# locuslab/qpth

Hardware: NVIDIA H100
Metric: QPs/sec (fwd+bwd) batch=128 nz=100 nineq=100 (higher is better)
Workload: dtype f64

## Files before the change

qpth_b200/csrc/qp_alt.cu:

```cuda
#include <cuda_runtime.h>
#include <math.h>
#include <stdint.h>
#include <string.h>

#include <mutex>

#include "../../include/qpth_b200.h"
#ifndef QPB_NT
#error "compile with -DQPB_NT=192|512 -DQPB_ALT_CTAS=3|1"
#endif
#define QPB_NS_CAT2(a, b) a##b
#define QPB_NS_CAT(a, b) QPB_NS_CAT2(a, b)
#define qpb QPB_NS_CAT(qpb_nt, QPB_NT)
#include "qp_solve.cuh"
#include "qp_setup_pf.cuh"

extern "C" void qpb200_internal_cuda_error(int err, const char* what);

namespace {

constexpr int kAltCtas = QPB_ALT_CTAS;
constexpr int kMin = (kAltCtas > 1) ? kAltCtas : 0;

KDims alt_dims(const qpb200_plan* p) {
    KDims D;
    D.n = p->nz; D.m = p->nineq; D.e = p->neq; D.ep = p->neq_pad; D.ms = p->ms; D.msp = p->ms_pad;
    D.ldw = p->ldw; D.lds = p->lds; D.rows_s = p->rows_s; D.vl = p->vl;
    D.lp = (int)p->L_elems;
    D.reg = 0.0;
    return D;
}

std::mutex g_mu;
template <typename K>
int alt_set_smem(K kernel, size_t bytes, size_t* cur) {
    int dev = 0;
    cudaError_t e = cudaGetDevice(&dev);
    if (e != cudaSuccess) { qpb200_internal_cuda_error((int)e, "cudaGetDevice"); return QPB200_ERR_CUDA; }
    std::lock_guard<std::mutex> lock(g_mu);
    if (dev < 16 && cur[dev] >= bytes) return QPB200_OK;
    e = cudaFuncSetAttribute(kernel, cudaFuncAttributeMaxDynamicSharedMemorySize, (int)bytes);
    if (e != cudaSuccess) { qpb200_internal_cuda_error((int)e, "cudaFuncSetAttribute"); return QPB200_ERR_CUDA; }
    if (dev < 16) cur[dev] = bytes;
    return QPB200_OK;
}
int alt_check_launch() {
    cudaError_t e = cudaGetLastError();
    if (e != cudaSuccess) { qpb200_internal_cuda_error((int)e, "kernel launch (qp_alt.cu)"); return QPB200_ERR_CUDA; }
    return QPB200_OK;
}
size_t g_fwd[16], g_kkt[16], g_bwd[16];

}

#define QPB_CAT2(a, b, c) a##b##c
#define QPB_CAT(a, b, c) QPB_CAT2(a, b, c)
#define QPB_ALT_NAME(fn) QPB_CAT(qpb200_alt, QPB_NT, fn)

extern "C" {

int QPB_ALT_NAME(_forward)(const qpb200_plan* plan, size_t smem, int nbatch, const double* p, int64_t sp, const double* h,
                           int64_t sh, const double* b, int64_t sb, const double* Lfac, const double* Wfac,
                           const double* Kfac, int sF, double eps, double stall_tol, double best_tie, int notImprovedLim,
                           int maxIter, double* zhat, double* lam, double* slacks, double* nus, int* iters,
                           double* best_resid, double* trace, void* stream) {
    cudaStream_t st = (cudaStream_t)stream;
    const KDims D = alt_dims(plan);
    int rc = alt_set_smem(k_forward_fast<true, true, kMin>, smem, g_fwd);
    if (rc) return rc;
    k_forward_fast<true, true, kMin><<<nbatch, qpb::fast::kNT, smem, st>>>(
        D, p, sp, h, sh, b, sb, Lfac, Wfac, Kfac, sF, eps, stall_tol, best_tie, notImprovedLim, maxIter, zhat, lam,
        slacks, nus, iters, best_resid, trace);
    return alt_check_launch();
}

int QPB_ALT_NAME(_forward_res)(const qpb200_plan* plan, size_t smem, int nbatch, const double* p, int64_t sp, const double* h,
                               int64_t sh, const double* b, int64_t sb, const double* Lfac, const double* Wfac,
                               const double* Kfac, int sF, double eps, double stall_tol, double best_tie, int notImprovedLim,
                               int maxIter, double* zhat, double* lam, double* slacks, double* nus, int* iters,
                               double* best_resid, double* trace, void* stream) {
#if QPB_NT == 512
    cudaStream_t st = (cudaStream_t)stream;
    const KDims D = alt_dims(plan);
    static size_t cur[16];
    int rc = alt_set_smem(k_forward_fast<false, true, 0>, smem, cur);
    if (rc) return rc;
    k_forward_fast<false, true, 0><<<nbatch, qpb::fast::kNT, smem, st>>>(
        D, p, sp, h, sh, b, sb, Lfac, Wfac, Kfac, sF, eps, stall_tol, best_tie, notImprovedLim, maxIter, zhat, lam,
        slacks, nus, iters, best_resid, trace);
    return alt_check_launch();
#else
    (void)plan; (void)smem; (void)nbatch; (void)p; (void)sp; (void)h; (void)sh; (void)b; (void)sb; (void)Lfac; (void)Wfac;
    (void)Kfac; (void)sF; (void)eps; (void)stall_tol; (void)best_tie; (void)notImprovedLim; (void)maxIter; (void)zhat;
    (void)lam; (void)slacks; (void)nus; (void)iters; (void)best_resid; (void)trace; (void)stream;
    return QPB200_ERR_BAD_ARG;
#endif
}

int QPB_ALT_NAME(_solve_kkt)(const qpb200_plan* plan, size_t smem, int nbatch, const double* d, const double* rx,
                             const double* rs, const double* rz, const double* ry, const double* Lfac, const double* Wfac,
                             const double* Kfac, int sF, double* dx, double* ds, double* dz, double* dy, void* stream) {
    cudaStream_t st = (cudaStream_t)stream;
    const KDims D = alt_dims(plan);
    BwdOut O;
    memset(&O, 0, sizeof(O));
    int rc = alt_set_smem(k_kkt_fast<false, true, true, kMin>, smem, g_kkt);
    if (rc) return rc;
    k_kkt_fast<false, true, true, kMin><<<nbatch, qpb::fast::kNT, smem, st>>>(
        D, d, rx, rs, rz, ry, nullptr, nullptr, nullptr, nullptr, Lfac, Wfac, Kfac, sF, dx, ds, dz, dy, O);
    return alt_check_launch();
}

#if QPB_NT == 192
int QPB_ALT_NAME(_setup)(const qpb200_plan* plan, size_t smem, int nsys, const double* Q, int64_t sQ, const double* G,
                         int64_t sG, const double* A, int64_t sA, double reg, double* Lfac, double* Wfac, double* Kfac,
                         int* spd_flag, void* stream) {
    static size_t g_setup[16];
    cudaStream_t st = (cudaStream_t)stream;
    KDims D = alt_dims(plan);
    D.reg = reg;
    int rc = alt_set_smem(k_setup_pf<kMin>, smem, g_setup);
    if (rc) return rc;
    k_setup_pf<kMin><<<nsys, qpb::fast::kNT, smem, st>>>(D, Q, sQ, G, sG, A, sA, Lfac, Wfac, Kfac, spd_flag);
    return alt_check_launch();
}
#endif

int QPB_ALT_NAME(_backward)(const qpb200_plan* plan, size_t smem, int nbatch, const double* dl_dzhat,
                            const double* dl_dlam, const double* dl_dnu, const double* zhat,
                            const double* lam, const double* slacks, const double* nus, const double* Lfac,
                            const double* Wfac, const double* Kfac, int sF, double* dQ, int mean_Q, double* dp, int mean_p,
                            double* dG, int mean_G, double* dh, int mean_h, double* dA, int mean_A, double* db, int mean_b,
                            double* dxv, double* dlamv, double* dnuv, void* stream) {
    cudaStream_t st = (cudaStream_t)stream;
    const KDims D = alt_dims(plan);
    BwdOut O;
    O.dQ = dQ; O.dp = dp; O.dG = dG; O.dh = dh; O.dA = dA; O.db = db;
    O.mQ = mean_Q; O.mp = mean_p; O.mG = mean_G; O.mh = mean_h; O.mA = mean_A; O.mb = mean_b;
    int rc = alt_set_smem(k_kkt_fast<true, true, true, kMin>, smem, g_bwd);
    if (rc) return rc;
    k_kkt_fast<true, true, true, kMin><<<nbatch, qpb::fast::kNT, smem, st>>>(
        D, nullptr, dl_dzhat, nullptr, dl_dlam, dl_dnu, zhat, lam, slacks, nus, Lfac, Wfac, Kfac, sF, dxv, nullptr,
        dlamv, dnuv, O);
    return alt_check_launch();
}

}
```

qpth_b200/csrc/qp_fast.cuh:

```cuda
#pragma once
#include "qp_device.cuh"

namespace qpb {
namespace fast {

#define QPB_SMEM extern __shared__ __align__(16) double qsm[]

#ifdef QPB_TIMING
__device__ long long g_cta[4 * 8192];
__device__ int g_tim_target = 0;
__device__ __forceinline__ long long gtimer() { long long t; asm volatile("mov.u64 %0, %globaltimer;" : "=l"(t)); return t; }
__device__ __forceinline__ int smid() { int r; asm volatile("mov.u32 %0, %smid;" : "=r"(r)); return r; }
__device__ long long g_tim[128];
__shared__ long long s_tim[129];
#define QPB_TICK(i)                                                         \
    do {                                                                    \
        if (threadIdx.x == 0) {                                             \
            const long long _t = clock64();                                 \
            s_tim[i] += _t - s_tim[128];                                    \
            s_tim[128] = _t;                                                \
        }                                                                   \
    } while (0)
__shared__ long long s_tim2;
#define QPB_TICK1(i)                                                        \
    do {                                                                    \
        if (threadIdx.x == 32) {                                            \
            const long long _t = clock64();                                 \
            s_tim[i] += _t - s_tim2;                                        \
            s_tim2 = _t;                                                    \
        }                                                                   \
    } while (0)
#else
#define QPB_TICK(i) do {} while (0)
#define QPB_TICK1(i) do {} while (0)
#endif

#ifndef QPB_NT
#define QPB_NT 256
#endif
constexpr int kNT = QPB_NT;


__device__ __forceinline__ void f_load_lower8(const double* Mb, int ld, double (&Lk)[36]) {
#pragma unroll
    for (int r = 0; r < 8; ++r)
#pragma unroll
        for (int c = 0; c <= r; c += 2) {
            const double2 v = *reinterpret_cast<const double2*>(Mb + r * ld + c);
            Lk[QPB_LIDX(r, c)] = v.x;
            if (c + 1 <= r) Lk[QPB_LIDX(r, c + 1)] = v.y;
        }
}

__device__ __forceinline__ double f_rsqrt(double x) {
    double y;
    asm("rsqrt.approx.ftz.f64 %0, %1;" : "=d"(y) : "d"(x));
    const double t = x * y;
    const double e = fma(-t, y, 1.0);
    const double p = fma(0.375, e, 0.5);
    const double ye = y * e;
    return fma(ye, p, y);
}

__device__ __forceinline__ void f_factor8_regs(double (&Lk)[36]) {
#pragma unroll
    for (int c = 0; c < 8; ++c) {
        const double ri = f_rsqrt(Lk[QPB_LIDX(c, c)]);
        Lk[QPB_LIDX(c, c)] = ri;
#pragma unroll
        for (int r = c + 1; r < 8; ++r) Lk[QPB_LIDX(r, c)] *= ri;
#pragma unroll
        for (int r = c + 1; r < 8; ++r)
#pragma unroll
            for (int cc = c + 1; cc <= r; ++cc)
                Lk[QPB_LIDX(r, cc)] = fma(-Lk[QPB_LIDX(r, c)], Lk[QPB_LIDX(cc, c)], Lk[QPB_LIDX(r, cc)]);
    }
}
__device__ __forceinline__ void f_store_lower8(double* Mb, int ld, const double (&Lk)[36]) {
#pragma unroll
    for (int r = 0; r < 8; ++r)
#pragma unroll
        for (int c = 0; c <= r; c += 2)
            *reinterpret_cast<double2*>(Mb + r * ld + c) =
                make_double2(Lk[QPB_LIDX(r, c)], (c + 1 <= r) ? Lk[QPB_LIDX(r, c + 1)] : 0.0);
}

__device__ __forceinline__ void f_row_solve8(double (&a)[8], const double (&Lk)[36]) {
#pragma unroll
    for (int c = 0; c < 8; ++c) {
        a[c] *= Lk[QPB_LIDX(c, c)];
#pragma unroll
        for (int c2 = c + 1; c2 < 8; ++c2) a[c2] = fma(-a[c], Lk[QPB_LIDX(c2, c)], a[c2]);
    }
}

__device__ __forceinline__ void f_ld8(const double* p, double (&a)[8]) {
    const double2 v0 = *reinterpret_cast<const double2*>(p), v1 = *reinterpret_cast<const double2*>(p + 2),
                  v2 = *reinterpret_cast<const double2*>(p + 4), v3 = *reinterpret_cast<const double2*>(p + 6);
    a[0] = v0.x; a[1] = v0.y; a[2] = v1.x; a[3] = v1.y; a[4] = v2.x; a[5] = v2.y; a[6] = v3.x; a[7] = v3.y;
}
__device__ __forceinline__ void f_st8(double* p, const double (&a)[8]) {
    *reinterpret_cast<double2*>(p) = make_double2(a[0], a[1]);
    *reinterpret_cast<double2*>(p + 2) = make_double2(a[2], a[3]);
    *reinterpret_cast<double2*>(p + 4) = make_double2(a[4], a[5]);
    *reinterpret_cast<double2*>(p + 6) = make_double2(a[6], a[7]);
}

__device__ __forceinline__ void named_bar_sync(int id, int count) {
    asm volatile("bar.sync %0, %1;" ::"r"(id), "r"(count) : "memory");
}
__device__ __forceinline__ void named_bar_arrive(int id, int count) {
    asm volatile("bar.arrive %0, %1;" ::"r"(id), "r"(count) : "memory");
}

__device__ __noinline__ void f_chol_chain(int A, int ld, int n, int c0) {
    QPB_SMEM;
    const int lane = threadIdx.x & 31;
    const int g = lane >> 2, q = lane & 3;
    const int nts = (n - c0) >> 3;
    double* M = qsm + A;
    double Lk[36];
    for (int k = -1; k < nts; ++k) {
        const int k0 = c0 + 8 * k;
        if (k >= 0 && k + 1 < nts) {
            if (lane < 8) {
                double a[8];
                double* rowp = M + (k0 + 8 + lane) * ld + k0;
                f_ld8(rowp, a);
                f_row_solve8(a, Lk);
                f_st8(rowp, a);
            }
            __syncwarp();
            named_bar_arrive(1, kNT);
            QPB_TICK(96 + k);
            double* pd = M + (k0 + 8 + g) * ld + k0 + 8 + 2 * q;
            const double* pr = M + (k0 + 8 + g) * ld + k0 + q;
            double2 cv = *reinterpret_cast<const double2*>(pd);
            const double a0 = pr[0], a1 = pr[4];
            dmma884(cv.x, cv.y, -a0, a0);
            dmma884(cv.x, cv.y, -a1, a1);
            *reinterpret_cast<double2*>(pd) = cv;
            __syncwarp();
            QPB_TICK(24);
        }
        if (k + 1 < nts) {
            f_load_lower8(M + (k0 + 8) * ld + k0 + 8, ld, Lk);
            __syncwarp();
            f_factor8_regs(Lk);
            if (lane == 0) f_store_lower8(M + (k0 + 8) * ld + k0 + 8, ld, Lk);
            if (k >= 0) QPB_TICK(80 + k);
        }
        QPB_TICK(26);
        __syncthreads();
        if (k >= 0) QPB_TICK(112 + k);
    }
}

__device__ __noinline__ void f_chol_update(int A, int ld, int n, int c0, int aug, int tabo) {
    QPB_SMEM;
    const int tid = threadIdx.x, lane = tid & 31, warp = tid >> 5;
    const int g = lane >> 2, q = lane & 3;
    const int nts = (n - c0) >> 3;
    const int noff = (nts * (nts - 1)) / 2;
    const uint16_t* tab = reinterpret_cast<const uint16_t*>(qsm + tabo);
    double* M = qsm + A;
    const int uw = (warp == 4) ? -1 : (warp < 4 ? warp - 1 : warp - 2);
    double C[kCholMaxOff][2];
    int tt_of[kCholMaxOff];
    const int gq = (c0 + g) * ld + q;
    if (uw >= 0) {
#pragma unroll
        for (int s = 0; s < kCholMaxOff; ++s) {
            const int idx = s * 6 + uw;
            const bool ok = idx < noff;
            const int tt = ok ? tab[idx] : 0;
            tt_of[s] = ok ? tt : -1;
            const double2 v = ok ? *reinterpret_cast<const double2*>(M + gq + q + 8 * (tt >> 8) * ld + c0 + 8 * (tt & 255))
                                 : make_double2(0.0, 0.0);
            C[s][0] = v.x; C[s][1] = v.y;
        }
    }
    __syncthreads();
    for (int k = 0; k < nts; ++k) {
        const int k0 = c0 + 8 * k;
        const bool last = (k + 1 >= nts);
        QPB_TICK1(40);
        {
            const int t = tid - 32;
            const int nrows = n - k0 - 16;
            const int naug = nrows > 0 ? nrows : 0;
            if (t <= naug) {
                double Ls[36], a[8];
                double* rowp = (t < naug) ? (M + (k0 + 16 + t) * ld + k0) : (qsm + aug + k0);
                f_ld8(rowp, a);
                f_load_lower8(M + k0 * ld + k0, ld, Ls);
                f_row_solve8(a, Ls);
                f_st8(rowp, a);
            }
        }
        QPB_TICK1(64 + k);
        if (!last) {
            named_bar_sync(1, kNT);
            QPB_TICK1(42);
            if (uw >= 0) {
#pragma unroll
                for (int s = kCholMaxOff - 1; s >= 0; s -= 2) {
                    const int s1 = s, s2 = (s - 1 >= 0) ? s - 1 : 0;
                    const int t1 = tt_of[s1], t2 = tt_of[s2];
                    const bool act1 = (t1 & 255) > k && t1 >= 0;
                    const bool act2 = (s - 1 >= 0) && (t2 & 255) > k && t2 >= 0;
                    if (!act1 && !act2) continue;
                    const double* pa1 = M + gq + 8 * (t1 >> 8) * ld + k0;
                    const double* pb1 = M + gq + 8 * (t1 & 255) * ld + k0;
                    const double* pa2 = M + gq + 8 * (t2 >> 8) * ld + k0;
                    const double* pb2 = M + gq + 8 * (t2 & 255) * ld + k0;
                    double a10 = 0, a11 = 0, b10 = 0, b11 = 0, a20 = 0, a21 = 0, b20 = 0, b21 = 0;
                    if (act1) { a10 = pa1[0]; a11 = pa1[4]; b10 = pb1[0]; b11 = pb1[4]; }
                    if (act2) { a20 = pa2[0]; a21 = pa2[4]; b20 = pb2[0]; b21 = pb2[4]; }
                    if (act1) dmma884(C[s1][0], C[s1][1], -a10, b10);
                    if (act2) dmma884(C[s2][0], C[s2][1], -a20, b20);
                    if (act1) dmma884(C[s1][0], C[s1][1], -a11, b11);
                    if (act2) dmma884(C[s2][0], C[s2][1], -a21, b21);
                    if (act1 && (t1 & 255) == k + 1)
                        *reinterpret_cast<double2*>(M + gq + q + 8 * (t1 >> 8) * ld + c0 + 8 * (k + 1)) = make_double2(C[s1][0], C[s1][1]);
                    if (act2 && (t2 & 255) == k + 1)
                        *reinterpret_cast<double2*>(M + gq + q + 8 * (t2 >> 8) * ld + c0 + 8 * (k + 1)) = make_double2(C[s2][0], C[s2][1]);
                }
                for (int s = k + 2 + uw; s < nts; s += 6) {
                    double* pd = M + (c0 + 8 * s + g) * ld + c0 + 8 * s + 2 * q;
                    const double* pr = M + (c0 + 8 * s + g) * ld + k0 + q;
                    double2 cv = *reinterpret_cast<const double2*>(pd);
                    const double a0 = pr[0], a1 = pr[4];
                    dmma884(cv.x, cv.y, -a0, a0);
                    dmma884(cv.x, cv.y, -a1, a1);
                    *reinterpret_cast<double2*>(pd) = cv;
                }
            } else {
                double y[8];
                f_ld8(qsm + aug + k0, y);
                for (int j = k0 + 8 + lane; j < n; j += 32) {
                    double pr[8];
                    f_ld8(M + j * ld + k0, pr);
                    double acc0 = qsm[aug + j], acc1 = 0.0;
#pragma unroll
                    for (int c = 0; c < 8; c += 2) { acc0 = fma(-pr[c], y[c], acc0); acc1 = fma(-pr[c + 1], y[c + 1], acc1); }
                    qsm[aug + j] = acc0 + acc1;
                }
            }
        }
        QPB_TICK1(48 + k);
        __syncthreads();
        QPB_TICK1(44);
    }
}

__device__ __forceinline__ void f_chol(int A, int ld, int n, int c0, int aug, int tabo) {
    if (threadIdx.x < 32) f_chol_chain(A, ld, n, c0);
    else f_chol_update(A, ld, n, c0, aug, tabo);
}

__device__ __noinline__ void f_trsv_fwd(int A, int ld, int n, int kbeg, int kend, int b, int u) {
    QPB_SMEM;
    const int tid = threadIdx.x;
    const double* M = qsm + A;
    for (int k0 = kbeg; k0 < kend; k0 += 8) {
        const int nbelow = n - k0 - 8;
        if (tid < nbelow || tid == 0) {
            double Lk[36], y[8], row[8];
            const bool has = tid < nbelow;
            f_ld8(qsm + b + k0, y);
            if (has) f_ld8(M + (k0 + 8 + tid) * ld + k0, row);
            f_load_lower8(M + k0 * ld + k0, ld, Lk);
            double acc0 = has ? qsm[b + k0 + 8 + tid] : 0.0, acc1 = 0.0;
#pragma unroll
            for (int c = 0; c < 8; ++c) {
                y[c] *= Lk[QPB_LIDX(c, c)];
#pragma unroll
                for (int c2 = c + 1; c2 < 8; ++c2) y[c2] = fma(-y[c], Lk[QPB_LIDX(c2, c)], y[c2]);
                if (has) { if (c & 1) acc1 = fma(-row[c], y[c], acc1); else acc0 = fma(-row[c], y[c], acc0); }
            }
            if (tid == 0) f_st8(qsm + u + k0, y);
            if (has) qsm[b + k0 + 8 + tid] = acc0 + acc1;
        }
        __syncthreads();
    }
}

__device__ __noinline__ void f_trsv_bwd(int A, int ld, int n, int u, int w) {
    QPB_SMEM;
    const int tid = threadIdx.x;
    const double* M = qsm + A;
    for (int k0 = n - 8; k0 >= 0; k0 -= 8) {
        if (tid < k0 || tid == 0) {
            double Lk[36], y[8];
            const bool has = tid < k0;
            f_ld8(qsm + u + k0, y);
            double col[8];
            if (has) {
#pragma unroll
                for (int c = 0; c < 8; ++c) col[c] = M[(k0 + c) * ld + tid];
            }
            f_load_lower8(M + k0 * ld + k0, ld, Lk);
            double acc0 = has ? qsm[u + tid] : 0.0, acc1 = 0.0;
#pragma unroll
            for (int c = 7; c >= 0; --c) {
                y[c] *= Lk[QPB_LIDX(c, c)];
#pragma unroll
                for (int c2 = 0; c2 < c; ++c2) y[c2] = fma(-y[c], Lk[QPB_LIDX(c, c2)], y[c2]);
                if (has) { if (c & 1) acc1 = fma(-col[c], y[c], acc1); else acc0 = fma(-col[c], y[c], acc0); }
            }
            if (tid == 0) f_st8(qsm + w + k0, y);
            if (has) qsm[u + tid] = acc0 + acc1;
        }
        __syncthreads();
    }
}

__device__ __noinline__ void f_invert8(int Mb_off, int ld) {
    QPB_SMEM;
    double* Mb = qsm + Mb_off;
    if ((threadIdx.x & 31) == 0) {
        double Lk[36], T[36];
        f_load_lower8(Mb, ld, Lk);
#pragma unroll
        for (int c = 0; c < 8; ++c) {
            T[QPB_LIDX(c, c)] = Lk[QPB_LIDX(c, c)];
#pragma unroll
            for (int r = c + 1; r < 8; ++r) {
                double sacc = 0.0;
#pragma unroll
                for (int j = c; j < r; ++j) sacc = fma(Lk[QPB_LIDX(r, j)], T[QPB_LIDX(j, c)], sacc);
                T[QPB_LIDX(r, c)] = -Lk[QPB_LIDX(r, r)] * sacc;
            }
        }
#pragma unroll
        for (int r = 1; r < 8; ++r)
#pragma unroll
            for (int c = 0; c < r; ++c) Mb[c * ld + r] = T[QPB_LIDX(r, c)];
    }
    __syncwarp();
}

__device__ __noinline__ void f_rows_times_LinvT(int A, int ld, int n, int Wm, int ldw, int rt) {
    QPB_SMEM;
    const int lane = threadIdx.x & 31, g = lane >> 2, q = lane & 3;
    const double* M = qsm + A;
    double* Wp = qsm + Wm + (8 * rt + g) * ldw;
    const int nct = n >> 3;
    for (int j = 0; j < nct; ++j) {
        double2 cv = *reinterpret_cast<const double2*>(Wp + 8 * j + 2 * q);
        const double* pb = M + (8 * j + g) * ld + q;
        for (int i = 0; i < j; ++i) {
            const double a0 = Wp[8 * i + q], a1 = Wp[8 * i + 4 + q];
            const double b0 = pb[8 * i], b1 = pb[8 * i + 4];
            dmma884(cv.x, cv.y, -a0, b0);
            dmma884(cv.x, cv.y, -a1, b1);
        }
        *reinterpret_cast<double2*>(Wp + 8 * j + 2 * q) = cv;
        __syncwarp();
        const double a0 = Wp[8 * j + q], a1 = Wp[8 * j + 4 + q];
        const double* Tb = M + (8 * j) * ld + 8 * j;
        const int c0 = q, c1 = 4 + q;
        const double b0 = (c0 < g) ? Tb[c0 * ld + g] : (c0 == g ? Tb[g * ld + g] : 0.0);
        const double b1 = (c1 < g) ? Tb[c1 * ld + g] : (c1 == g ? Tb[g * ld + g] : 0.0);
        double d0 = 0.0, d1 = 0.0;
        dmma884(d0, d1, a0, b0);
        dmma884(d0, d1, a1, b1);
        __syncwarp();
        *reinterpret_cast<double2*>(Wp + 8 * j + 2 * q) = make_double2(d0, d1);
        __syncwarp();
    }
}

__device__ __noinline__ void f_whiten(int Lp, int n, int dinvL, int b, int u) {
    QPB_SMEM;
    trsv_fwd(qsm + Lp, PackedIdx{}, n, 0, n, qsm + dinvL, qsm + b, qsm + u, (int)threadIdx.x, kNT);
}
__device__ __noinline__ void f_unwhiten(int Lp, int n, int dinvL, int u, int w) {
    QPB_SMEM;
    trsv_bwd(qsm + Lp, PackedIdx{}, n, qsm + dinvL, qsm + u, qsm + w, (int)threadIdx.x, kNT);
}

template <bool kTwo>
__device__ __forceinline__ void f_matvec_rows_impl(int W, int ld, int rows, int cols, int x1, int x2, int y1, int y2) {
    QPB_SMEM;
    const int tid = threadIdx.x, h = tid & 1;
    for (int rb = 0; rb < rows; rb += kNT / 2) {
        const int r = rb + (tid >> 1);
        const bool ok = r < rows;
        const double* a = qsm + W + (ok ? r : 0) * ld + 2 * h;
        double s1a = 0.0, s1b = 0.0, s2a = 0.0, s2b = 0.0;
#pragma unroll 2
        for (int c = 2 * h; c < cols; c += 4, a += 4) {
            const double2 w = *reinterpret_cast<const double2*>(a);
            const double2 u = *reinterpret_cast<const double2*>(qsm + x1 + c);
            const bool hi = c + 1 < cols;
            const double wy = hi ? w.y : 0.0;
            s1a = fma(w.x, u.x, s1a); s1b = fma(wy, hi ? u.y : 0.0, s1b);
            if (kTwo) {
                const double2 v = *reinterpret_cast<const double2*>(qsm + x2 + c);
                s2a = fma(w.x, v.x, s2a); s2b = fma(wy, hi ? v.y : 0.0, s2b);
            }
        }
        double s1 = s1a + s1b, s2 = s2a + s2b;
        __syncwarp();
        s1 += __shfl_xor_sync(0xffffffffu, s1, 1);
        if (kTwo) s2 += __shfl_xor_sync(0xffffffffu, s2, 1);
        if (ok && h == 0) {
            qsm[y1 + r] = s1;
            if (kTwo) qsm[y2 + r] = s2;
        }
    }
}
__device__ __noinline__ void f_matvec_rows2(int W, int ld, int rows, int cols, int x1, int x2, int y1, int y2) {
    f_matvec_rows_impl<true>(W, ld, rows, cols, x1, x2, y1, y2);
}
__device__ __noinline__ void f_matvec_rows1(int W, int ld, int rows, int cols, int x1, int y1) {
    f_matvec_rows_impl<false>(W, ld, rows, cols, x1, 0, y1, 0);
}
__device__ __noinline__ void f_matvec_cols(int W, int ld, int rows, int cols, int v, int p0, int p1, int out,
                                           int a, double sa, int b, double sgn) {
    QPB_SMEM;
    const int tid = threadIdx.x;
    const int half = kNT / 2;
    const int gidx = tid / half, c = tid - gidx * half;
    const int chunk = (rows + 1) >> 1;
    for (int c0 = 0; c0 < cols; c0 += half) {
        const int cc = c0 + c;
        if (cc < cols) {
            const int r0 = gidx * chunk, r1 = min(rows, r0 + chunk);
            const double* Wp = qsm + W + cc;
            double s0 = 0.0, s1 = 0.0, s2 = 0.0, s3 = 0.0;
            int r = r0;
#pragma unroll 1
            for (; r + 3 < r1; r += 4) {
                s0 = fma(Wp[(r + 0) * ld], qsm[v + r + 0], s0);
                s1 = fma(Wp[(r + 1) * ld], qsm[v + r + 1], s1);
                s2 = fma(Wp[(r + 2) * ld], qsm[v + r + 2], s2);
                s3 = fma(Wp[(r + 3) * ld], qsm[v + r + 3], s3);
            }
#pragma unroll 1
            for (; r < r1; ++r) s0 = fma(Wp[r * ld], qsm[v + r], s0);
            qsm[(gidx ? p1 : p0) + cc] = (s0 + s1) + (s2 + s3);
        }
    }
    __syncthreads();
    for (int cc = tid; cc < cols; cc += kNT) {
        double r = sa * qsm[a + cc] + sgn * (qsm[p0 + cc] + qsm[p1 + cc]);
        if (b >= 0) r += qsm[b + cc];
        qsm[out + cc] = r;
    }
    __syncthreads();
}

__device__ __forceinline__ void f_cols2_out(int c, double wdv, double wv, int xt, int rxt, int pt, double alpha) {
    QPB_SMEM;
    const double dx = -qsm[rxt + c] - wdv;
    const double x = fma(alpha, dx, qsm[xt + c]);
    qsm[xt + c] = x;
    qsm[rxt + c] = (x + wv) + qsm[pt + c];
}
__device__ __noinline__ void f_matvec_cols2(int W, int ld, int rows, int cols, int dv, int v, int p0, int p1, int p2,
                                            int p3, int xt, int rxt, int pt, double alpha) {
    QPB_SMEM;
    const int tid = threadIdx.x;
    const int half = kNT / 2;
    const int gidx = tid / half, c = tid - gidx * half;
    const int chunk = (rows + 1) >> 1;
    for (int c0 = 0; c0 < cols; c0 += half) {
        const int cc = c0 + c;
        if (cc < cols) {
            const int r0 = gidx * chunk, r1 = min(rows, r0 + chunk);
            const double* Wp = qsm + W + cc;
            double s0 = 0.0, s1 = 0.0, s2 = 0.0, s3 = 0.0, u0 = 0.0, u1 = 0.0, u2 = 0.0, u3 = 0.0;
            int r = r0;
#pragma unroll 1
            for (; r + 3 < r1; r += 4) {
                const double w0 = Wp[(r + 0) * ld], w1 = Wp[(r + 1) * ld], w2 = Wp[(r + 2) * ld], w3 = Wp[(r + 3) * ld];
                s0 = fma(w0, qsm[dv + r + 0], s0); u0 = fma(w0, qsm[v + r + 0], u0);
                s1 = fma(w1, qsm[dv + r + 1], s1); u1 = fma(w1, qsm[v + r + 1], u1);
                s2 = fma(w2, qsm[dv + r + 2], s2); u2 = fma(w2, qsm[v + r + 2], u2);
                s3 = fma(w3, qsm[dv + r + 3], s3); u3 = fma(w3, qsm[v + r + 3], u3);
            }
#pragma unroll 1
            for (; r < r1; ++r) {
                const double w0 = Wp[r * ld];
                s0 = fma(w0, qsm[dv + r], s0); u0 = fma(w0, qsm[v + r], u0);
            }
            qsm[(gidx ? p1 : p0) + cc] = (s0 + s1) + (s2 + s3);
            qsm[(gidx ? p3 : p2) + cc] = (u0 + u1) + (u2 + u3);
        }
    }
    __syncthreads();
    for (int cc = tid; cc < cols; cc += kNT)
        f_cols2_out(cc, qsm[p0 + cc] + qsm[p1 + cc], qsm[p2 + cc] + qsm[p3 + cc], xt, rxt, pt, alpha);
    __syncthreads();
}

__device__ __noinline__ double f_tri_norm2(int Lp, int n, int x) {
    QPB_SMEM;
    const int tid = threadIdx.x, q4 = tid >> 2, l = tid & 3;
    double acc = 0.0;
    const int npairs = (n + 1) >> 1;
    for (int pb = 0; pb < npairs; pb += kNT / 4) {
        const int pi = pb + q4;
        const bool act = pi < npairs;
        const int ra = act ? pi : 0, rb = n - 1 - ra;
        const double* La = qsm + Lp + (ra * (ra + 1)) / 2;
        const double* Lb = qsm + Lp + (rb * (rb + 1)) / 2;
        double sa = 0.0, sb = 0.0;
        if (act) {
#pragma unroll 2
            for (int c = l; c <= ra; c += 4) sa = fma(La[c], qsm[x + c], sa);
            if (rb != ra) {
#pragma unroll 2
                for (int c = l; c <= rb; c += 4) sb = fma(Lb[c], qsm[x + c], sb);
            }
        }
        __syncwarp();
        sa += __shfl_xor_sync(0xffffffffu, sa, 1); sb += __shfl_xor_sync(0xffffffffu, sb, 1);
        sa += __shfl_xor_sync(0xffffffffu, sa, 2); sb += __shfl_xor_sync(0xffffffffu, sb, 2);
        if (l == 0) acc = fma(sa, sa, fma(sb, sb, acc));
    }
    return acc;
}

__device__ __forceinline__ double2 ldg2(const double* p) { return __ldg(reinterpret_cast<const double2*>(p)); }

template <bool kTwo>
__device__ __forceinline__ void g_matvec_rows_impl(const double* __restrict__ Wg, int ld, int rows, int cols, int x1,
                                                   int x2, int y1, int y2) {
    QPB_SMEM;
    constexpr int kRG = kNT / 8;
    const int tid = threadIdx.x, j = tid & 7, rg = kRG - 1 - (tid >> 3);
#pragma unroll 1
    for (int rb = 0; rb < rows; rb += 2 * kRG) {
        const int r0 = rb + rg, r1 = r0 + kRG;
        const bool ok0 = r0 < rows, ok1 = r1 < rows;
        const double* p0 = Wg + (size_t)(ok0 ? r0 : 0) * ld;
        const double* p1 = Wg + (size_t)(ok1 ? r1 : 0) * ld;
        double a0 = 0.0, a1 = 0.0, b0 = 0.0, b1 = 0.0;
#pragma unroll 1
        for (int cb = 2 * j; cb < cols; cb += 112) {
            double2 w0[7], w1[7];
#pragma unroll
            for (int k = 0; k < 7; ++k) {
                const int c = cb + 16 * k;
                const bool in = c < cols;
                w0[k] = in ? ldg2(p0 + c) : make_double2(0.0, 0.0);
                w1[k] = in ? ldg2(p1 + c) : make_double2(0.0, 0.0);
            }
#pragma unroll
            for (int k = 0; k < 7; ++k) {
                const int c = cb + 16 * k;
                if (c < cols) {
                    const bool hi = c + 1 < cols;
                    double2 u = *reinterpret_cast<const double2*>(qsm + x1 + c);
                    if (!hi) u.y = 0.0;
                    const double wy0 = hi ? w0[k].y : 0.0, wy1 = hi ? w1[k].y : 0.0;
                    a0 = fma(w0[k].x, u.x, a0); a0 = fma(wy0, u.y, a0);
                    b0 = fma(w1[k].x, u.x, b0); b0 = fma(wy1, u.y, b0);
                    if (kTwo) {
                        double2 v = *reinterpret_cast<const double2*>(qsm + x2 + c);
                        if (!hi) v.y = 0.0;
                        a1 = fma(w0[k].x, v.x, a1); a1 = fma(wy0, v.y, a1);
                        b1 = fma(w1[k].x, v.x, b1); b1 = fma(wy1, v.y, b1);
                    }
                }
            }
        }
        __syncwarp();
#pragma unroll
        for (int o = 1; o < 8; o <<= 1) {
            a0 += __shfl_xor_sync(0xffffffffu, a0, o);
            b0 += __shfl_xor_sync(0xffffffffu, b0, o);
            if (kTwo) {
                a1 += __shfl_xor_sync(0xffffffffu, a1, o);
                b1 += __shfl_xor_sync(0xffffffffu, b1, o);
            }
        }
        if (j == 0) {
            if (ok0) { qsm[y1 + r0] = a0; if (kTwo) qsm[y2 + r0] = a1; }
            if (ok1) { qsm[y1 + r1] = b0; if (kTwo) qsm[y2 + r1] = b1; }
        }
    }
}
__device__ __noinline__ void g_matvec_rows2(const double* __restrict__ Wg, int ld, int rows, int cols, int x1, int x2,
                                            int y1, int y2) {
    g_matvec_rows_impl<true>(Wg, ld, rows, cols, x1, x2, y1, y2);
}
__device__ __noinline__ void g_matvec_rows1(const double* __restrict__ Wg, int ld, int rows, int cols, int x1, int y1) {
    g_matvec_rows_impl<false>(Wg, ld, rows, cols, x1, 0, y1, 0);
}

__device__ __noinline__ void g_matvec_cols(const double* __restrict__ Wg, int ld, int rows, int cols, int v, int out,
                                           int a, double sa, int b, double sgn) {
    QPB_SMEM;
    const int tid = threadIdx.x, lane = tid & 31, warp = tid >> 5, g = lane >> 3, cq = lane & 7;
#pragma unroll 1
    for (int c0 = 0; c0 < cols; c0 += 16 * (kNT / 32)) {
        const int c = c0 + 16 * warp + 2 * cq;
        const bool okc = c < cols;
        const double* pc = Wg + (okc ? c : 0);
        double s0 = 0.0, s1 = 0.0;
#pragma unroll 1
        for (int rb = g; rb < rows; rb += 4 * 13) {
            double2 w[13];
#pragma unroll
            for (int k = 0; k < 13; ++k) {
                const int r = rb + 4 * k;
                w[k] = (r < rows) ? ldg2(pc + (size_t)r * ld) : make_double2(0.0, 0.0);
            }
#pragma unroll
            for (int k = 0; k < 13; ++k) {
                const int r = rb + 4 * k;
                if (r < rows) {
                    const double vr = qsm[v + r];
                    s0 = fma(w[k].x, vr, s0);
                    s1 = fma(w[k].y, vr, s1);
                }
            }
        }
        __syncwarp();
        s0 += __shfl_xor_sync(0xffffffffu, s0, 8);  s1 += __shfl_xor_sync(0xffffffffu, s1, 8);
        s0 += __shfl_xor_sync(0xffffffffu, s0, 16); s1 += __shfl_xor_sync(0xffffffffu, s1, 16);
        if (g == 0 && okc) {
            double r0 = sa * qsm[a + c] + sgn * s0;
            if (b >= 0) r0 += qsm[b + c];
            qsm[out + c] = r0;
            if (c + 1 < cols) {
                double r1 = sa * qsm[a + c + 1] + sgn * s1;
                if (b >= 0) r1 += qsm[b + c + 1];
                qsm[out + c + 1] = r1;
            }
        }
    }
    __syncthreads();
}

__device__ __noinline__ void g_matvec_cols2(const double* __restrict__ Wg, int ld, int rows, int cols, int dv, int v,
                                            int xt, int rxt, int pt, double alpha) {
    QPB_SMEM;
    const int tid = threadIdx.x, lane = tid & 31, warp = tid >> 5, g = lane >> 3, cq = lane & 7;
#pragma unroll 1
    for (int c0 = 0; c0 < cols; c0 += 16 * (kNT / 32)) {
        const int c = c0 + 16 * warp + 2 * cq;
        const bool okc = c < cols;
        const double* pc = Wg + (okc ? c : 0);
        double s0 = 0.0, s1 = 0.0, u0 = 0.0, u1 = 0.0;
#pragma unroll 1
        for (int rb = g; rb < rows; rb += 4 * 13) {
            double2 w[13];
#pragma unroll
            for (int k = 0; k < 13; ++k) {
                const int r = rb + 4 * k;
                w[k] = (r < rows) ? ldg2(pc + (size_t)r * ld) : make_double2(0.0, 0.0);
            }
#pragma unroll
            for (int k = 0; k < 13; ++k) {
                const int r = rb + 4 * k;
                if (r < rows) {
                    const double dr = qsm[dv + r], vr = qsm[v + r];
                    s0 = fma(w[k].x, dr, s0);
                    s1 = fma(w[k].y, dr, s1);
                    u0 = fma(w[k].x, vr, u0);
                    u1 = fma(w[k].y, vr, u1);
                }
            }
        }
        __syncwarp();
        s0 += __shfl_xor_sync(0xffffffffu, s0, 8);  s1 += __shfl_xor_sync(0xffffffffu, s1, 8);
        u0 += __shfl_xor_sync(0xffffffffu, u0, 8);  u1 += __shfl_xor_sync(0xffffffffu, u1, 8);
        s0 += __shfl_xor_sync(0xffffffffu, s0, 16); s1 += __shfl_xor_sync(0xffffffffu, s1, 16);
        u0 += __shfl_xor_sync(0xffffffffu, u0, 16); u1 += __shfl_xor_sync(0xffffffffu, u1, 16);
        if (g == 0 && okc) {
            f_cols2_out(c, s0, u0, xt, rxt, pt, alpha);
            if (c + 1 < cols) f_cols2_out(c + 1, s1, u1, xt, rxt, pt, alpha);
        }
    }
    __syncthreads();
}

__device__ __noinline__ double g_tri_norm2(const double* __restrict__ Lg, int n, int x) {
    QPB_SMEM;
    const int tid = threadIdx.x, q4 = tid >> 2, l = tid & 3;
    double acc = 0.0;
    const int npairs = (n + 1) >> 1;
    for (int pb = 0; pb < npairs; pb += kNT / 4) {
        const int pi = pb + q4;
        const bool act = pi < npairs;
        const int ra = act ? pi : 0, rb = n - 1 - ra;
        const double* La = Lg + (ra * (ra + 1)) / 2;
        const double* Lb = Lg + (rb * (rb + 1)) / 2;
        double sa = 0.0, sb = 0.0;
        if (act) {
#pragma unroll 1
            for (int cb = l; cb <= rb; cb += 4 * 13) {
                double wa[13], wb[13];
#pragma unroll
                for (int k = 0; k < 13; ++k) {
                    const int c = cb + 4 * k;
                    wb[k] = (c <= rb) ? __ldg(Lb + c) : 0.0;
                    wa[k] = (c <= ra && rb != ra) ? __ldg(La + c) : 0.0;
                }
#pragma unroll
                for (int k = 0; k < 13; ++k) {
                    const int c = cb + 4 * k;
                    if (c <= rb) {
                        const double xc = qsm[x + c];
                        sb = fma(wb[k], xc, sb);
                        sa = fma(wa[k], xc, sa);
                    }
                }
            }
        }
        __syncwarp();
        sa += __shfl_xor_sync(0xffffffffu, sa, 1); sb += __shfl_xor_sync(0xffffffffu, sb, 1);
        sa += __shfl_xor_sync(0xffffffffu, sa, 2); sb += __shfl_xor_sync(0xffffffffu, sb, 2);
        if (l == 0) acc = fma(sa, sa, fma(sb, sb, acc));
    }
    return acc;
}

constexpr int kFastStride = (kNT / 32 <= 8) ? 8 : 16;
__device__ __noinline__ void f_reduce_sum4(double (&v)[4], int red) {
    QPB_SMEM;
    block_reduce<4, false, kFastStride>(v, qsm + red, (int)threadIdx.x, kNT);
}
__device__ __noinline__ void f_reduce_sum2(double (&v)[2], int red) {
    QPB_SMEM;
    block_reduce<2, false, kFastStride>(v, qsm + red, (int)threadIdx.x, kNT);
}
__device__ __noinline__ void f_reduce_min2(double (&v)[2], int red) {
    QPB_SMEM;
    block_reduce<2, true, kFastStride>(v, qsm + red, (int)threadIdx.x, kNT);
}

}
}
```

Measured before the change: 311,800.

## Rebalance narrow-column W products and flatten triangular norm loads

```diff
diff --git a/qpth_b200/csrc/qp_alt.cu b/qpth_b200/csrc/qp_alt.cu
--- a/qpth_b200/csrc/qp_alt.cu
+++ b/qpth_b200/csrc/qp_alt.cu
@@ -145,4 +145,25 @@
     return alt_check_launch();
 }
 
+#ifdef QPB_TIMING
+int QPB_ALT_NAME(_debug_timing)(long long* host64, int reset) {
+    cudaError_t e;
+    if (reset) {
+        long long z[128] = {0};
+        const int target = reset >= 2 ? reset - 2 : 0;
+        e = cudaMemcpyToSymbol(qpb::fast::g_tim, z, sizeof(z));
+        if (e == cudaSuccess) e = cudaMemcpyToSymbol(qpb::fast::g_tim_target, &target, sizeof(int));
+    } else {
+        e = cudaMemcpyFromSymbol(host64, qpb::fast::g_tim, 128 * sizeof(long long));
+    }
+    if (e != cudaSuccess) { qpb200_internal_cuda_error((int)e, "debug_timing (qp_alt.cu)"); return QPB200_ERR_CUDA; }
+    return QPB200_OK;
 }
+int QPB_ALT_NAME(_debug_cta)(long long* host64, int nqp) {
+    cudaError_t e = cudaMemcpyFromSymbol(host64, qpb::fast::g_cta, (size_t)4 * nqp * sizeof(long long));
+    if (e != cudaSuccess) { qpb200_internal_cuda_error((int)e, "debug_cta (qp_alt.cu)"); return QPB200_ERR_CUDA; }
+    return QPB200_OK;
+}
+#endif
+
+}
diff --git a/qpth_b200/csrc/qp_fast.cuh b/qpth_b200/csrc/qp_fast.cuh
--- a/qpth_b200/csrc/qp_fast.cuh
+++ b/qpth_b200/csrc/qp_fast.cuh
@@ -12,20 +12,20 @@
 __device__ __forceinline__ long long gtimer() { long long t; asm volatile("mov.u64 %0, %globaltimer;" : "=l"(t)); return t; }
 __device__ __forceinline__ int smid() { int r; asm volatile("mov.u32 %0, %smid;" : "=r"(r)); return r; }
 __device__ long long g_tim[128];
-__shared__ long long s_tim[129];
+__shared__ unsigned s_tim[129];
 #define QPB_TICK(i)                                                         \
     do {                                                                    \
         if (threadIdx.x == 0) {                                             \
-            const long long _t = clock64();                                 \
+            const unsigned _t = (unsigned)clock64();                        \
             s_tim[i] += _t - s_tim[128];                                    \
             s_tim[128] = _t;                                                \
         }                                                                   \
     } while (0)
-__shared__ long long s_tim2;
+__shared__ unsigned s_tim2;
 #define QPB_TICK1(i)                                                        \
     do {                                                                    \
         if (threadIdx.x == 32) {                                            \
-            const long long _t = clock64();                                 \
+            const unsigned _t = (unsigned)clock64();                        \
             s_tim[i] += _t - s_tim2;                                        \
             s_tim2 = _t;                                                    \
         }                                                                   \
@@ -644,27 +644,65 @@
     const int tid = threadIdx.x, lane = tid & 31, warp = tid >> 5, g = lane >> 3, cq = lane & 7;
 #pragma unroll 1
     for (int c0 = 0; c0 < cols; c0 += 16 * (kNT / 32)) {
-        const int c = c0 + 16 * warp + 2 * cq;
+        const int cw = c0 + 16 * warp;
+        if (cw >= cols) continue;
+        const int npw = min(8, (cols - cw + 1) >> 1);
+        const int c = cw + 2 * cq;
         const bool okc = c < cols;
-        const double* pc = Wg + (okc ? c : 0);
         double s0 = 0.0, s1 = 0.0, u0 = 0.0, u1 = 0.0;
-#pragma unroll 1
-        for (int rb = g; rb < rows; rb += 4 * 13) {
-            double2 w[13];
-#pragma unroll
-            for (int k = 0; k < 13; ++k) {
-                const int r = rb + 4 * k;
-                w[k] = (r < rows) ? ldg2(pc + (size_t)r * ld) : make_double2(0.0, 0.0);
-            }
-#pragma unroll
-            for (int k = 0; k < 13; ++k) {
-                const int r = rb + 4 * k;
-                if (r < rows) {
-                    const double dr = qsm[dv + r], vr = qsm[v + r];
-                    s0 = fma(w[k].x, dr, s0);
-                    s1 = fma(w[k].y, dr, s1);
-                    u0 = fma(w[k].x, vr, u0);
-                    u1 = fma(w[k].y, vr, u1);
+        if (npw > 2) {
+            const double* pc = Wg + (okc ? c : 0);
+#pragma unroll 1
+            for (int rb = g; rb < rows; rb += 4 * 13) {
+                double2 w[13];
+#pragma unroll
+                for (int k = 0; k < 13; ++k) {
+                    const int r = rb + 4 * k;
+                    w[k] = (r < rows) ? ldg2(pc + (size_t)r * ld) : make_double2(0.0, 0.0);
+                }
+#pragma unroll
+                for (int k = 0; k < 13; ++k) {
+                    const int r = rb + 4 * k;
+                    if (r < rows) {
+                        const double dr = qsm[dv + r], vr = qsm[v + r];
+                        s0 = fma(w[k].x, dr, s0);
+                        s1 = fma(w[k].y, dr, s1);
+                        u0 = fma(w[k].x, vr, u0);
+                        u1 = fma(w[k].y, vr, u1);
+                    }
+                }
+            }
+        } else {
+            const int tg = (rows > g ? ((rows - g + 3) >> 2) : 0) * npw;
+            const int tmax = ((rows + 3) >> 2) * npw;
+            const int src = lane & 24;
+#pragma unroll 1
+            for (int tb = 0; tb < tmax; tb += 8 * 7) {
+                double2 w[7];
+#pragma unroll
+                for (int k = 0; k < 7; ++k) {
+                    const int t = tb + 8 * k + cq;
+                    const int kr = (npw == 2) ? (t >> 1) : t;
+                    w[k] = (t < tg) ? ldg2(Wg + (size_t)(g + 4 * kr) * ld + cw + 2 * (t - kr * npw)) : make_double2(0.0, 0.0);
+                }
+#pragma unroll
+                for (int k = 0; k < 7; ++k) {
+                    if (tb + 8 * k >= tmax) break;
+#pragma unroll 1
+                    for (int jj = 0; jj < 8; ++jj) {
+                        const double wx = __shfl_sync(0xffffffffu, w[k].x, src | jj);
+                        const double wy = __shfl_sync(0xffffffffu, w[k].y, src | jj);
+                        const int t = tb + 8 * k + jj;
+                        const int kr = (npw == 2) ? (t >> 1) : t;
+                        if (t < tg && cq == t - kr * npw) {
+                            const int r = g + 4 * kr;
+                            const double dr = qsm[dv + r], vr = qsm[v + r];
+                            s0 = fma(wx, dr, s0);
+                            s1 = fma(wy, dr, s1);
+                            u0 = fma(wx, vr, u0);
+                            u1 = fma(wy, vr, u1);
+                        }
+                    }
                 }
             }
         }
@@ -690,27 +728,28 @@
         const int pi = pb + q4;
         const bool act = pi < npairs;
         const int ra = act ? pi : 0, rb = n - 1 - ra;
-        const double* La = Lg + (ra * (ra + 1)) / 2;
-        const double* Lb = Lg + (rb * (rb + 1)) / 2;
+        const double* La = Lg + (ra * (ra + 1)) / 2 + l;
+        const double* Lb = Lg + (rb * (rb + 1)) / 2 + l;
+        const int na = (act && rb != ra && l <= ra) ? ((ra - l) >> 2) + 1 : 0;
+        const int nt = act && l <= rb ? na + ((rb - l) >> 2) + 1 : 0;
+        const double* Lb0 = Lb - 4 * na;
         double sa = 0.0, sb = 0.0;
-        if (act) {
-#pragma unroll 1
-            for (int cb = l; cb <= rb; cb += 4 * 13) {
-                double wa[13], wb[13];
-#pragma unroll
-                for (int k = 0; k < 13; ++k) {
-                    const int c = cb + 4 * k;
-                    wb[k] = (c <= rb) ? __ldg(Lb + c) : 0.0;
-                    wa[k] = (c <= ra && rb != ra) ? __ldg(La + c) : 0.0;
-                }
-#pragma unroll
-                for (int k = 0; k < 13; ++k) {
-                    const int c = cb + 4 * k;
-                    if (c <= rb) {
-                        const double xc = qsm[x + c];
-                        sb = fma(wb[k], xc, sb);
-                        sa = fma(wa[k], xc, sa);
-                    }
+#pragma unroll 1
+        for (int t0 = 0; t0 < nt; t0 += 26) {
+            double w[26];
+#pragma unroll
+            for (int k = 0; k < 26; ++k) {
+                const int t = t0 + k;
+                w[k] = (t < nt) ? __ldg((t < na ? La : Lb0) + 4 * t) : 0.0;
+            }
+#pragma unroll
+            for (int k = 0; k < 26; ++k) {
+                const int t = t0 + k;
+                if (t < nt) {
+                    const bool ia = t < na;
+                    const double xc = qsm[x + l + 4 * (ia ? t : t - na)];
+                    if (ia) sa = fma(w[k], xc, sa);
+                    else sb = fma(w[k], xc, sb);
                 }
             }
         }
```

Measured after the change: 294,400, median of 6. 5.6% lower.
